# fbergama/wass

Hardware: AMD Instinct MI355X
Metric: stereo_pairs_per_sec (higher is better)
Workload: dtype u16

## Files before the change

### wass_amd/build.py

```python
from __future__ import annotations

import glob
import os
import subprocess
import sys

_HERE = os.path.dirname(os.path.abspath(__file__))
CSRC = os.path.join(_HERE, "csrc")
OBJ = os.path.join(CSRC, "_obj")
SO = os.path.join(_HERE, "libwassgpu.so")
HIPCC = os.environ.get("HIPCC", "/opt/rocm/bin/hipcc")
FLAGS = ["--offload-arch=gfx950", "-O3", "-std=c++17", "-fPIC", "-ffp-contract=off", "-Wall",
         "-Wno-unused-function", "-fno-gpu-rdc"] + os.environ.get("WASS_EXTRA_FLAGS", "").split()


def _newer(src: str, dst: str, deps) -> bool:
    if not os.path.exists(dst):
        return True
    t = os.path.getmtime(dst)
    return any(os.path.getmtime(p) > t for p in [src, *deps])


def build(force: bool = False, verbose: bool = False) -> str:
    os.makedirs(OBJ, exist_ok=True)
    srcs = sorted(glob.glob(os.path.join(CSRC, "*.hip")))
    deps = sorted(glob.glob(os.path.join(CSRC, "*.h"))) + [os.path.join(_HERE, "..", "include", "wass_gpu.h")]
    stamp = os.path.join(OBJ, ".flags")
    try:
        hipcc_version = subprocess.run([HIPCC, "--version"], capture_output=True, text=True).stdout.strip().replace("\n", " | ")
    except OSError:
        hipcc_version = "?"
    flags_now = " ".join(FLAGS) + " || " + hipcc_version
    try:
        same = open(stamp).read() == flags_now
    except OSError:
        same = False
    if not same:
        force = True
        for stale in (stamp, SO):
            try:
                os.remove(stale)
            except OSError:
                pass
    objs, procs = [], []
    for s in srcs:
        o = os.path.join(OBJ, os.path.basename(s)[:-4] + ".o")
        objs.append(o)
        if force or _newer(s, o, deps):
            cmd = [HIPCC, *FLAGS, "-c", s, "-o", o]
            if verbose:
                print(" ".join(cmd))
            procs.append((s, subprocess.Popen(cmd)))
    failed = [s for s, p in procs if p.wait() != 0]
    if failed:
        raise RuntimeError("hipcc failed for: " + ", ".join(failed))
    if force or procs or not os.path.exists(SO):
        cmd = [HIPCC, "--offload-arch=gfx950", "-shared", "-fPIC", "-o", SO, *objs, "-ldl"]
        if verbose:
            print(" ".join(cmd))
        subprocess.check_call(cmd)
    with open(stamp, "w") as f:
        f.write(flags_now)
    return SO


HOST_DIR = os.path.join(_HERE, "host")
BIN_DIR = os.path.join(_HERE, "bin")
CLI = os.path.join(BIN_DIR, "wass_stereo")
CLI_GPU = os.path.join(BIN_DIR, "wass_stereo_gpu")
BATCH = os.path.join(BIN_DIR, "wass_stereo_batch")
PREPARE = os.path.join(BIN_DIR, "wass_prepare")


def build_host(force: bool = False, verbose: bool = False) -> str:
    build(force=False)
    os.makedirs(BIN_DIR, exist_ok=True)
    deps = sorted(glob.glob(os.path.join(HOST_DIR, "*.hpp"))) + [os.path.join(_HERE, "..", "include", "wass_gpu.h"), SO]
    for name, exe in (("wass_stereo_client.cpp", CLI), ("wass_stereo.cpp", CLI_GPU), ("wass_stereo_batch.cpp", BATCH), ("wass_prepare.cpp", PREPARE)):
        src = os.path.join(HOST_DIR, name)
        if force or _newer(src, exe, deps):
            cmd = [os.environ.get("CXX", "g++"), "-O2", "-std=c++17", "-Wall", "-Wno-unused-function", src, "-o", exe]
            if exe != CLI:
                cmd += ["-L" + _HERE, "-lwassgpu", "-lz", "-pthread", "-Wl,-rpath,$ORIGIN/..", "-Wl,-rpath-link," + "/opt/rocm/lib"]
            if verbose:
                print(" ".join(cmd))
            subprocess.check_call(cmd)
    return CLI


if __name__ == "__main__":
    print(build(force="--force" in sys.argv, verbose=True))
    print(build_host(force="--force" in sys.argv, verbose=True))
```

### wass_amd/csrc/sgm_aggregate.hip

```cpp
#include "sgm_step.h"

namespace wass {

template <int NP, int SMODE, int U>
__global__ void __launch_bounds__(256) k_sweep(const uint32_t* __restrict__ C, uint32_t* __restrict__ S,
                                               int width1, int h, int dx, int dy, int P1, int P2, int nchains, int D,
                                               int minD, int uniq, int keepS, int16_t* __restrict__ sel_d16,
                                               uint32_t* __restrict__ sel_key)
{
    const int lane = threadIdx.x & 63;
    const int c = blockIdx.x * 4 + __builtin_amdgcn_readfirstlane(threadIdx.x >> 6);
    if (c >= nchains) return;
    int x0, y0, n;
    chain_geometry(c, dx, dy, width1, h, x0, y0, n);
    const long long vec = 64 * NP;
    const long long step = ((long long)dy * width1 + dx) * vec;
    const long long pixstep = (long long)dy * width1 + dx;
    long long pix = (long long)y0 * width1 + x0;
    const uint32_t* cp = C + pix * vec + lane * NP;
    uint32_t* sp = S + pix * vec + lane * NP;
    const us2 P1v = pk_splat(P1), cap = pk_splat(0x7FFF);

    auto finish = [&](const us2 (&L)[NP], const us2 (&sin)[NP], uint32_t* so, us2 (&sv)[NP]) {
#pragma unroll
        for (int j = 0; j < NP; ++j) sv[j] = SMODE == 0 ? pk_min(L[j], cap) : pk_min(pk_adds(sin[j], L[j]), cap);
        if (SMODE != 2 || keepS) {
            st_stream_vec<NP>(so, sv);
        }
    };

    PathState<NP> st;
    st.reset();
    const int F = n / U, r = n - F * U;
    us2 cb[U][NP], sb[U][NP], cn[U][NP], sn[U][NP];
    if (F > 0) {
        load_seg<NP, U, false>(cp, step, U, cb);
        if (SMODE != 0) load_seg<NP, U, false>(sp, step, U, sb);
    }
    for (int g = 0; g < F; ++g) {
        if (g + 1 < F) {
            load_seg<NP, U, false>(cp + U * step, step, U, cn);
            if (SMODE != 0) load_seg<NP, U, false>(sp + U * step, step, U, sn);
        }
        us2 fin[U][NP];
#pragma unroll
        for (int u = 0; u < U; ++u) {
            us2 L[NP];
            sgm_step<NP>(st, cb[u], L, P1v, P2);
            finish(L, sb[u], sp + u * step, fin[u]);
        }
        if (SMODE == 2) wta_batch<NP, U>(fin, U, lane, D, minD, uniq, sel_d16, sel_key, pix, pixstep);
        copy_seg<NP, U>(cb, cn);
        if (SMODE != 0) copy_seg<NP, U>(sb, sn);
        cp += U * step;
        sp += U * step;
        pix += U * pixstep;
    }
    if (r > 0) {
        load_seg<NP, U, true>(cp, step, r, cb);
        if (SMODE != 0) load_seg<NP, U, true>(sp, step, r, sb);
        us2 fin[U][NP];
#pragma unroll
        for (int u = 0; u < U; ++u) {
#pragma unroll
            for (int j = 0; j < NP; ++j) fin[u][j] = cap;
            if (u < r) {
                us2 L[NP];
                sgm_step<NP>(st, cb[u], L, P1v, P2);
                finish(L, sb[u], sp + u * step, fin[u]);
            }
        }
        if (SMODE == 2) wta_batch<NP, U>(fin, r, lane, D, minD, uniq, sel_d16, sel_key, pix, pixstep);
    }
}

#ifndef WASS_CKPT_WAVES
#define WASS_CKPT_WAVES 3
#endif
template <int NP, int K>
__global__ void __launch_bounds__(256) __attribute__((amdgpu_waves_per_eu(1, WASS_CKPT_WAVES))) k_ckpt(const uint32_t* __restrict__ C, uint32_t* __restrict__ ckpt,
                                              uint16_t* __restrict__ mins, int width1, int h, int dx, int dy, int P1, int P2,
                                              int nchains, int maxseg, uint32_t* __restrict__ endstate)
{
    const int lane = threadIdx.x & 63;
    const int c = blockIdx.x * 4 + __builtin_amdgcn_readfirstlane(threadIdx.x >> 6);
    if (c >= nchains) return;
    int x0, y0, n;
    if (endstate) half_chain_geometry(c, dx, dy, width1, h, x0, y0, n);
    else chain_geometry(c, dx, dy, width1, h, x0, y0, n);
    constexpr int VB = 256 * NP;
    const long long vec = 64 * NP;
    ChainAddr a;
    a.pixstep = (long long)dy * width1 + dx;
    a.pix0 = (long long)y0 * width1 + x0;
    a.sstep = (int)a.pixstep * VB;
    const uint32_t voff = lane * NP * 4;
    const uint32_t bK = a.bias(K);
    const us2 P1v = pk_splat(P1);
    const int F = n / K, r = n - F * K;
    const int ncp = endstate ? F : F - (r > 0 ? 0 : 1);
    const rsrc_t ckr = mk_rsrc(ckpt + (long long)c * maxseg * vec);
    uint32_t* mrow = (uint32_t*)(mins + (size_t)c * maxseg * K);

    PathState<NP> st;
    st.reset();
    us2 ring[K][NP];
    if (ncp > 0) {
        const rsrc_t r0 = a.run<NP>(C, 0, K);
#pragma unroll
        for (int u = 0; u < K; ++u) buf_ld<NP>(r0, voff, bK + u * a.sstep, ring[u]);
    }
    for (int s = 0; s < ncp; ++s) {
        uint32_t ms[K];
        const rsrc_t rn = a.run<NP>(C, (long long)min(s + 1, F - 1) * K, K);
#pragma unroll
        for (int u = 0; u < K; ++u) {
            us2 L[NP];
            sgm_step<NP>(st, ring[u], L, P1v, P2);
            ms[u] = st.m;
            buf_ld<NP>(rn, voff, bK + u * a.sstep, ring[u]);
        }
        {
            const us2 mvv = pk_splat(st.m);
            us2 nrm[NP];
#pragma unroll
            for (int j = 0; j < NP; ++j) nrm[j] = st.L[j] - mvv;
            buf_st<NP>(ckr, voff, (uint32_t)s * VB, nrm);
        }
        store_minima<K>(mrow + (size_t)s * (K / 2), ms, lane);
    }
    if (endstate) {
        if (r > 0) {
            const rsrc_t rt = a.run<NP>(C, (long long)F * K, r);
            const uint32_t br = a.bias(r);
#pragma unroll
            for (int u = 0; u < K; ++u)
                if (u < r) buf_ld<NP>(rt, voff, br + u * a.sstep, ring[u]);
#pragma unroll
            for (int u = 0; u < K; ++u)
                if (u < r) {
                    us2 L[NP];
                    sgm_step<NP>(st, ring[u], L, P1v, P2);
                }
        }
        st.store_normalised(endstate + (long long)c * vec + lane * NP);
    }
}

template <int NP>
__device__ __forceinline__ void lds_st(uint32_t* p, const us2 (&v)[NP])
{
    if constexpr (NP % 4 == 0) {
#pragma unroll
        for (int j = 0; j < NP; j += 4) *(wass_u32x4*)(p + j) = wass_u32x4{ as_u32(v[j]), as_u32(v[j + 1]), as_u32(v[j + 2]), as_u32(v[j + 3]) };
    } else if constexpr (NP % 2 == 0) {
#pragma unroll
        for (int j = 0; j < NP; j += 2) *(wass_u32x2*)(p + j) = wass_u32x2{ as_u32(v[j]), as_u32(v[j + 1]) };
    } else {
#pragma unroll
        for (int j = 0; j < NP; ++j) p[j] = as_u32(v[j]);
    }
}
template <int NP>
__device__ __forceinline__ void lds_ld(const uint32_t* p, us2 (&v)[NP])
{
    if constexpr (NP % 4 == 0) {
#pragma unroll
        for (int j = 0; j < NP; j += 4) {
            const wass_u32x4 t = *(const wass_u32x4*)(p + j);
            v[j] = as_us2(t.x); v[j + 1] = as_us2(t.y); v[j + 2] = as_us2(t.z); v[j + 3] = as_us2(t.w);
        }
    } else if constexpr (NP % 2 == 0) {
#pragma unroll
        for (int j = 0; j < NP; j += 2) {
            const wass_u32x2 t = *(const wass_u32x2*)(p + j);
            v[j] = as_us2(t.x); v[j + 1] = as_us2(t.y);
        }
    } else {
#pragma unroll
        for (int j = 0; j < NP; ++j) v[j] = as_us2(p[j]);
    }
}

#ifndef WASS_VREC
#define WASS_VREC 7
#endif
#ifndef WASS_REC_TIE
#define WASS_REC_TIE 0
#endif
#ifndef WASS_REC_FENCE
#define WASS_REC_FENCE 1
#endif
template <int N, bool VEC>
struct Rec {
    uint32_t v[VEC ? 1 : N / 2];
    __device__ __forceinline__ void clear()
    {
#pragma unroll
        for (int i = 0; i < (VEC ? 1 : N / 2); ++i) v[i] = 0;
    }
    __device__ __forceinline__ void load(const uint32_t* p, int lane)
    {
        if constexpr (VEC) {
            v[0] = __builtin_amdgcn_raw_buffer_load_b32(mk_rsrc(p), (uint32_t)min(lane, N / 2 - 1) * 4u, 0, 0);
#if WASS_REC_TIE
            asm volatile("" : "+v"(v[0]) :: "memory");
#elif WASS_REC_FENCE
            asm volatile("" ::: "memory");
#endif
        } else {
#pragma unroll
            for (int i = 0; i < N / 2; ++i) v[i] = p[i];
        }
    }
    __device__ __forceinline__ uint32_t at(int i) const
    {
        if constexpr (VEC) return (__builtin_amdgcn_readlane(v[0], i >> 1) >> ((i & 1) * 16)) & 0xFFFFu;
        else return (v[i >> 1] >> ((i & 1) * 16)) & 0xFFFFu;
    }
    __device__ __forceinline__ uint32_t at_dyn(int i) const
    {
        uint32_t w;
        if constexpr (VEC) w = __builtin_amdgcn_readlane(v[0], i >> 1);
        else {
            w = v[0];
#pragma unroll
            for (int k = 1; k < N / 2; ++k) w = (i >> 1) == k ? v[k] : w;
        }
        return (w >> ((i & 1) * 16)) & 0xFFFFu;
    }
    __device__ __forceinline__ uint32_t before(int u) const { return u == 0 ? 0u : at(u - 1); }
};

#ifndef WASS_PAIR_WAVES
#define WASS_PAIR_WAVES 4
#endif
template <int NP, int K, int SMODE>
__global__ void __launch_bounds__(256) __attribute__((amdgpu_waves_per_eu(WASS_PAIR_WAVES, WASS_PAIR_WAVES)))
k_pair(const uint32_t* __restrict__ C, uint32_t* __restrict__ S, const uint32_t* __restrict__ ckpt,
       const uint16_t* __restrict__ mins, int width1, int h, int dx, int dy, int P1, int P2, int nchains, int maxseg, int D,
       int minD, int uniq, int keepS, int16_t* __restrict__ sel_d16, uint32_t* __restrict__ sel_key,
       const uint32_t* __restrict__ endstate)
{
    static_assert(K % 2 == 0, "the minima records are read as dwords");
    constexpr int VW = 64 * NP;
    __shared__ __attribute__((aligned(16))) uint32_t hand[4][2][K][VW];
    const int lane = threadIdx.x & 63;
    const int wv = __builtin_amdgcn_readfirstlane(threadIdx.x >> 6);
    const int c = blockIdx.x * 4 + wv;
    if (c >= nchains) return;
    int x0, y0, n;
    if (endstate) half_chain_geometry(c, dx, dy, width1, h, x0, y0, n);
    else chain_geometry(c, dx, dy, width1, h, x0, y0, n);
    constexpr int VB = 256 * NP;
    constexpr bool LAST = SMODE == 2;
    const long long vec = VW;
    ChainAddr a;
    a.pixstep = (long long)dy * width1 + dx;
    a.pix0 = (long long)y0 * width1 + x0;
    a.sstep = (int)a.pixstep * VB;
    const uint32_t voff = lane * NP * 4;
    const uint32_t bK = a.bias(K);
    const us2 P1v = pk_splat(P1), cap = pk_splat(0x7FFF);
    const int F = n / K, r = n - F * K;
    const rsrc_t ckr = mk_rsrc(ckpt + (long long)c * maxseg * vec);
    const uint32_t* mrow = (const uint32_t*)(mins + (size_t)c * maxseg * K);
    uint32_t* hc = &hand[wv][0][0][lane * NP];
    uint32_t* hl = &hand[wv][1][0][lane * NP];

    PathState<NP> bw;
    bw.reset();
    if (endstate) {
        us2 nv[NP];
        ld_stream_vec<NP>(endstate + (long long)(c ^ 1) * vec + lane * NP, nv);
        bw.load_normalised(nv);
    }
    auto finish = [&](const us2 (&lf)[NP], const us2 (&lb)[NP], const us2 (&sin)[NP], us2 (&sv)[NP]) {
#pragma unroll
        for (int j = 0; j < NP; ++j) {
            const us2 both = pk_adds(lf[j], lb[j]);
            const us2 acc = SMODE == 0 ? both : pk_adds(sin[j], both);
            sv[j] = LAST ? pk_min(acc, cap) : acc;
        }
    };
    if (r > 0) {
        const rsrc_t rc = a.run<NP>(C, (long long)F * K, r), rs = a.run<NP>(S, (long long)F * K, r);
        const uint32_t br = a.bias(r);
        us2 cb[K][NP], lf[K][NP], sb[K][NP];
#pragma unroll
        for (int u = 0; u < K; ++u)
            if (u < r) {
                buf_ld<NP>(rc, voff, br + u * a.sstep, cb[u]);
                if (SMODE != 0) buf_ld<NP>(rs, voff, br + u * a.sstep, sb[u]);
            }
        PathState<NP> fw;
        fw.reset();
        if (F > 0) {
            us2 nv[NP];
            buf_ld<NP>(ckr, voff, (uint32_t)(F - 1) * VB, nv);
            fw.load_normalised(nv);
        }
#pragma unroll
        for (int u = 0; u < K; ++u)
            if (u < r) sgm_step<NP>(fw, cb[u], lf[u], P1v, P2);
        us2 fin[K][NP];
#pragma unroll
        for (int u = K - 1; u >= 0; --u) {
#pragma unroll
            for (int j = 0; j < NP; ++j) fin[u][j] = cap;
            if (u < r) {
                us2 L[NP];
                sgm_step<NP>(bw, cb[u], L, P1v, P2);
                finish(lf[u], L, sb[u], fin[u]);
                if (!LAST || keepS) buf_st<NP>(rs, voff, br + u * a.sstep, fin[u]);
            }
        }
        if (LAST) wta_batch<NP, K>(fin, r, lane, D, minD, uniq, sel_d16, sel_key, a.pix0 + (long long)F * K * a.pixstep, a.pixstep);
    }
    if (F == 0) return;

    us2 cf[K][NP], sr[K][NP];
    PathState<NP> fw;
    us2 nvB[NP];
    Rec<K, (WASS_VREC & 1) != 0> mB;
    mB.clear();
    {
        const int s = F - 1;
        const rsrc_t rc = a.run<NP>(C, (long long)s * K, K), rs = a.run<NP>(S, (long long)s * K, K);
        const rsrc_t rc2 = a.run<NP>(C, (long long)max(s - 1, 0) * K, K);
        if (s >= 2) buf_ld<NP>(ckr, voff, (uint32_t)(s - 2) * VB, nvB);
        else {
#pragma unroll
            for (int j = 0; j < NP; ++j) nvB[j] = pk_splat(0);
        }
        mB.load(mrow + (size_t)max(s - 1, 0) * (K / 2), lane);
        us2 c0[K][NP];
        fw.reset();
        us2 nv[NP];
        if (s >= 1) buf_ld<NP>(ckr, voff, (uint32_t)(s - 1) * VB, nv);
#pragma unroll
        for (int u = 0; u < K; ++u) {
            buf_ld<NP>(rc, voff, bK + u * a.sstep, c0[u]);
            if (SMODE != 0) buf_ld<NP>(rs, voff, bK + u * a.sstep, sr[u]);
        }
#pragma unroll
        for (int u = 0; u < K; ++u) buf_ld<NP>(rc2, voff, bK + u * a.sstep, cf[u]);
        if (s >= 1) fw.load_normalised(nv);
#pragma unroll
        for (int u = 0; u < K; ++u) {
            us2 L[NP];
            sgm_step<NP>(fw, c0[u], L, P1v, P2);
            lds_st<NP>(hc + u * VW, c0[u]);
            lds_st<NP>(hl + u * VW, L);
        }
    }

    us2 fin[K][NP];
    bool odd = false;
    int s = F - 1;
    __builtin_amdgcn_s_waitcnt(0x0F70);
    while (s >= 1) {
        const rsrc_t rcN = a.run<NP>(C, (long long)max(s - 2, 0) * K, K);
        const rsrc_t rsN = a.run<NP>(S, (long long)(s - 1) * K, K), rsO = a.run<NP>(S, (long long)s * K, K);
        us2 nvC[NP];
        Rec<K, (WASS_VREC & 1) != 0> mC;
        if (s >= 3) buf_ld<NP>(ckr, voff, (uint32_t)(s - 3) * VB, nvC);
        else {
#pragma unroll
            for (int j = 0; j < NP; ++j) nvC[j] = pk_splat(0);
        }
        mC.load(mrow + (size_t)max(s - 2, 0) * (K / 2), lane);
        fw.load_normalised(nvB);
        const int stp = odd ? VW : -VW;
        uint32_t* pc = hc + (odd ? 0 : (K - 1) * VW);
        us2 cbn[NP], lfn[NP];
        lds_ld<NP>(pc, cbn);
        lds_ld<NP>(pc + K * VW, lfn);
#pragma unroll
        for (int u = 0; u < K; ++u) {
            const int v = K - 1 - u;
            uint32_t* pn = pc + stp;
            us2 cb[NP], lfv[NP], Lf[NP], Lb[NP], sv[NP];
#pragma unroll
            for (int j = 0; j < NP; ++j) { cb[j] = cbn[j]; lfv[j] = lfn[j]; }
            if (u + 1 < K) {
                lds_ld<NP>(pn, cbn);
                lds_ld<NP>(pn + K * VW, lfn);
            }
            sgm_step_fb<NP>(fw, mB.before(u), cf[u], Lf, bw, cb, Lb, P1v, P2);
            finish(lfv, Lb, sr[v], sv);
            if (!LAST || keepS) buf_st<NP>(rsO, voff, bK + v * a.sstep, sv);
            if (LAST) {
#pragma unroll
                for (int j = 0; j < NP; ++j) fin[v][j] = sv[j];
            }
            lds_st<NP>(pc, cf[u]);
            lds_st<NP>(pc + K * VW, Lf);
            buf_ld<NP>(rcN, voff, bK + u * a.sstep, cf[u]);
            if (SMODE != 0) buf_ld<NP>(rsN, voff, bK + v * a.sstep, sr[v]);
            pc = pn;
        }
        if (LAST) wta_batch<NP, K>(fin, K, lane, D, minD, uniq, sel_d16, sel_key, a.pix0 + (long long)s * K * a.pixstep, a.pixstep);
#pragma unroll
        for (int j = 0; j < NP; ++j) nvB[j] = nvC[j];
        mB = mC;
        odd = !odd;
        --s;
    }
    {
        const rsrc_t rsO = a.run<NP>(S, 0, K);
        const int stp = odd ? VW : -VW;
        uint32_t* pc = hc + (odd ? 0 : (K - 1) * VW);
#pragma unroll
        for (int u = 0; u < K; ++u) {
            const int v = K - 1 - u;
            us2 cb[NP], lfv[NP], Lb[NP], sv[NP];
            lds_ld<NP>(pc, cb);
            lds_ld<NP>(pc + K * VW, lfv);
            sgm_step<NP>(bw, cb, Lb, P1v, P2);
            finish(lfv, Lb, sr[v], sv);
            if (!LAST || keepS) buf_st<NP>(rsO, voff, bK + v * a.sstep, sv);
            if (LAST) {
#pragma unroll
                for (int j = 0; j < NP; ++j) fin[v][j] = sv[j];
            }
            pc += stp;
        }
        if (LAST) wta_batch<NP, K>(fin, K, lane, D, minD, uniq, sel_d16, sel_key, a.pix0, a.pixstep);
    }
}

#ifndef WASS_FUSE_NP
#define WASS_FUSE_NP 4
#endif
template <int NP> struct Fuse {
    static constexpr int XB = NP <= 3 ? 10 : 8;
    static constexpr int MINW = NP <= 2 ? 5 : 2;
    static constexpr int MAXW = NP <= 2 ? 5 : (NP == 3 ? 3 : 2);
};
inline int fuse_xb(int NP) { return NP <= 3 ? 10 : 8; }

template <int NP>
__global__ void __launch_bounds__(256) __attribute__((amdgpu_waves_per_eu(1, 4)))
k_rowsweep(const uint32_t* __restrict__ C, uint32_t* __restrict__ entF, uint32_t* __restrict__ entB, uint16_t* __restrict__ MF,
           uint16_t* __restrict__ MB, int width1, int h, int P1, int P2, int nbx)
{
    constexpr int XB = Fuse<NP>::XB;
    const int lane = threadIdx.x & 63;
    const int y = blockIdx.x * 4 + __builtin_amdgcn_readfirstlane(threadIdx.x >> 6);
    if (y >= h) return;
    constexpr int VB = 256 * NP;
    const long long vec = 64 * NP;
    const int n = width1;
    ChainAddr af, ab;
    af.pixstep = 1;  af.pix0 = (long long)y * width1;           af.sstep = VB;
    ab.pixstep = -1; ab.pix0 = (long long)y * width1 + n - 1;   ab.sstep = -VB;
    const uint32_t voff = lane * NP * 4;
    const us2 P1v = pk_splat(P1);
    const int cb = n % XB;
    uint32_t* mfrow = (uint32_t*)(MF + (size_t)y * nbx * XB);
    uint16_t* mbrow = MB + (size_t)y * nbx * XB;
    uint32_t* efrow = entF + (size_t)y * nbx * vec + lane * NP;
    uint32_t* ebrow = entB + (size_t)y * nbx * vec + lane * NP;

    PathState<NP> sf, sb;
    sf.reset();
    sb.reset();
    us2 rf[XB][NP], rb[XB][NP];
    const int G = n / XB, rem = n - G * XB;
    if (G > 0) {
        const rsrc_t r0 = af.run<NP>(C, 0, XB), r1 = ab.run<NP>(C, 0, XB);
        const uint32_t b1 = ab.bias(XB);
#pragma unroll
        for (int u = 0; u < XB; ++u) {
            buf_ld<NP>(r0, voff, u * VB, rf[u]);
            buf_ld<NP>(r1, voff, b1 + u * ab.sstep, rb[u]);
        }
        __builtin_amdgcn_s_waitcnt(0x0F70);
    }
    for (int g = 0; g < G; ++g) {
        const int t0 = g * XB;
        const int nxt = min(t0 + XB, n - 1), cnn = min(XB, n - nxt);
        const rsrc_t rnf = af.run<NP>(C, nxt, cnn), rnb = ab.run<NP>(C, nxt, cnn);
        const uint32_t bnb = ab.bias(cnn);
        uint32_t msf[XB], msb[XB];
#pragma unroll
        for (int u = 0; u < XB; ++u) {
            const int t = t0 + u;
            if (u == 0 && g > 0) sf.store_normalised(efrow + (size_t)g * vec);
            if (u == cb && t > 0) sb.store_normalised(ebrow + (size_t)((n - 1 - t) / XB) * vec);
            us2 Lf[NP], Lb[NP];
            sgm_step_pair<NP>(sf, rf[u], Lf, sb, rb[u], Lb, P1v, P2);
            msf[u] = sf.m;
            msb[XB - 1 - u] = sb.m;
            const int uc = min(u, cnn - 1);
            buf_ld<NP>(rnf, voff, uc * VB, rf[u]);
            buf_ld<NP>(rnb, voff, bnb + uc * ab.sstep, rb[u]);
        }
        store_minima<XB>(mfrow + (size_t)g * (XB / 2), msf, lane);
        {
            uint32_t v = msb[0];
#pragma unroll
            for (int i = 1; i < XB; ++i) v = lane == i ? msb[i] : v;
            if (lane < XB) mbrow[n - t0 - XB + lane] = (uint16_t)v;
        }
    }
    if (rem > 0) {
        const int t0 = G * XB;
        if (G == 0) {
            const rsrc_t r0 = af.run<NP>(C, 0, rem), r1 = ab.run<NP>(C, 0, rem);
            const uint32_t b1 = ab.bias(rem);
#pragma unroll
            for (int u = 0; u < XB; ++u)
                if (u < rem) {
                    buf_ld<NP>(r0, voff, u * VB, rf[u]);
                    buf_ld<NP>(r1, voff, b1 + u * ab.sstep, rb[u]);
                }
        }
        uint32_t msf[XB], msb[XB];
#pragma unroll
        for (int i = 0; i < XB; ++i) msf[i] = msb[i] = 0;
#pragma unroll
        for (int u = 0; u < XB; ++u)
            if (u < rem) {
                const int t = t0 + u;
                if (u == 0 && G > 0) sf.store_normalised(efrow + (size_t)G * vec);
                if (u == cb && t > 0) sb.store_normalised(ebrow + (size_t)((n - 1 - t) / XB) * vec);
                us2 Lf[NP], Lb[NP];
                sgm_step_pair<NP>(sf, rf[u], Lf, sb, rb[u], Lb, P1v, P2);
                msf[u] = sf.m;
#pragma unroll
                for (int i = 0; i < XB; ++i) msb[i] = i == rem - 1 - u ? sb.m : msb[i];
            }
        store_minima<XB>(mfrow + (size_t)G * (XB / 2), msf, lane);
        {
            uint32_t v = msb[0];
#pragma unroll
            for (int i = 1; i < XB; ++i) v = lane == i ? msb[i] : v;
            if (lane < rem) mbrow[lane] = (uint16_t)v;
        }
    }
}

struct RowSide {
    const uint32_t* entF; const uint32_t* entB;
    const uint16_t* MF; const uint16_t* MB;
    int nbx;
};

template <int NP, int K, bool ACC, bool ONE>
__global__ void __launch_bounds__(64 * Fuse<NP>::XB) __attribute__((amdgpu_waves_per_eu(Fuse<NP>::MINW, Fuse<NP>::MAXW)))
k_pairx(const uint32_t* __restrict__ C, uint32_t* __restrict__ S, const uint32_t* __restrict__ ckpt, const uint16_t* __restrict__ mins,
        const RowSide rs, int width1, int h, int P1, int P2, int maxseg, const uint32_t* __restrict__ endstate)
{
    constexpr int XB = Fuse<NP>::XB;
    static_assert(K % 2 == 0 && K <= XB && XB % 2 == 0, "one wave per row of a K-row segment; minima records are read as dwords");
    static_assert((size_t)XB * 2 * K * 256 * NP <= 160 * 1024, "the hand-over block must fit a CU's LDS");
    constexpr int VW = 64 * NP, VB = 256 * NP;
    extern __shared__ __attribute__((aligned(16))) uint32_t hand_raw[];
    constexpr int SS = XB * VW;
    constexpr int KS = K * XB * VW;
    const int lane = threadIdx.x & 63;
    const int wv = __builtin_amdgcn_readfirstlane(threadIdx.x >> 6);
    const int bx = blockIdx.x >> 1, half = blockIdx.x & 1;
    const uint32_t keepF = (!ONE || half == 0) ? 0xFFFFFFFFu : 0u, keepB = (!ONE || half == 1) ? 0xFFFFFFFFu : 0u;
    auto drop = [](us2 (&v)[NP], uint32_t keep) {
        if constexpr (ONE) {
#pragma unroll
            for (int j = 0; j < NP; ++j) v[j] = as_us2(as_u32(v[j]) & keep);
        }
    };
    const int X0 = bx * XB, ncol = min(XB, width1 - X0);
    const bool colact = wv < ncol;
    const int x = colact ? X0 + wv : X0;
    const int c = 2 * x + half;
    int dx = 0, dy = 1, x0, y0, n;
    half_chain_geometry(c, dx, dy, width1, h, x0, y0, n);
    if (n == 0) return;
    const long long vec = VW;
    ChainAddr a;
    a.pixstep = (long long)dy * width1;
// ... 490 lines not shown
```

### wass_amd/csrc/sgm_step.h

```cpp
#pragma once

#include "common.h"

namespace wass {

#ifndef WASS_NT
#define WASS_NT 1
#endif
__device__ __forceinline__ uint32_t ld_stream(const uint32_t* p)
{
#if WASS_NT
    return __builtin_nontemporal_load(p);
#else
    return *p;
#endif
}
__device__ __forceinline__ void st_stream(uint32_t* p, uint32_t v)
{
#if WASS_NT
    __builtin_nontemporal_store(v, p);
#else
    *p = v;
#endif
}
// ... 227 lines not shown
}

template <int K>
__device__ __forceinline__ void store_minima(uint32_t* __restrict__ rec, const uint32_t (&ms)[K], int lane)
{
    static_assert(K % 2 == 0, "records are dwords");
    uint32_t v = ms[0] | (ms[1] << 16);
#pragma unroll
    for (int i = 1; i < K / 2; ++i) v = lane == i ? (ms[2 * i] | (ms[2 * i + 1] << 16)) : v;
    if (lane < K / 2) rec[lane] = v;
}

template <int NP>
__device__ __forceinline__ void sgm_step_fb(PathState<NP>& a, const uint32_t am, const us2 (&ca)[NP], us2 (&La)[NP],
                                            PathState<NP>& b, const us2 (&cb)[NP], us2 (&Lb)[NP],
                                            const us2 P1v, const uint32_t P2)
{
    a.shr = dpp_mov<DPP_WAVE_SHR1>(a.shr, as_u32(a.L[NP - 1]));
    b.shr = dpp_mov<DPP_WAVE_SHR1>(b.shr, as_u32(b.L[NP - 1]));
    a.shl = dpp_mov<DPP_WAVE_SHL1>(a.shl, as_u32(a.L[0]));
    b.shl = dpp_mov<DPP_WAVE_SHL1>(b.shl, as_u32(b.L[0]));
    const us2 amv = pk_splat(am), amp2 = pk_splat(am + P2);
    const us2 bmv = pk_splat(b.m), bmp2 = pk_splat(b.m + P2);
#pragma unroll
    for (int j = 0; j < NP; ++j) {
        const uint32_t alo = j == 0 ? a.shr : as_u32(a.L[j - 1]);
        const uint32_t blo = j == 0 ? b.shr : as_u32(b.L[j - 1]);
        const uint32_t ahi = j == NP - 1 ? a.shl : as_u32(a.L[j + 1]);
        const uint32_t bhi = j == NP - 1 ? b.shl : as_u32(b.L[j + 1]);
        const us2 anl = as_us2(__builtin_amdgcn_alignbit(as_u32(a.L[j]), alo, 16));
        const us2 bnl = as_us2(__builtin_amdgcn_alignbit(as_u32(b.L[j]), blo, 16));
        const us2 anr = as_us2(__builtin_amdgcn_alignbit(ahi, as_u32(a.L[j]), 16));
        const us2 bnr = as_us2(__builtin_amdgcn_alignbit(bhi, as_u32(b.L[j]), 16));
        us2 ax = pk_min(anl, anr);
        us2 bx = pk_min(bnl, bnr);
        ax = pk_adds(ax, P1v);
        bx = pk_adds(bx, P1v);
        ax = pk_min(a.L[j], ax);
        bx = pk_min(b.L[j], bx);
        ax = pk_min(ax, amp2);
        bx = pk_min(bx, bmp2);
        ax = ax - amv;
        bx = bx - bmv;
        La[j] = pk_adds(ca[j], ax);
        Lb[j] = pk_adds(cb[j], bx);
    }
    us2 bm = Lb[0];
#pragma unroll
    for (int j = 1; j < NP; ++j) bm = pk_min(bm, Lb[j]);
    b.m = wave_min_u32(min((uint32_t)bm.x, (uint32_t)bm.y));
#pragma unroll
    for (int j = 0; j < NP; ++j) { a.L[j] = La[j]; b.L[j] = Lb[j]; }
}

template <int NP>
__device__ __forceinline__ void sgm_step_ff(PathState<NP>& a, const uint32_t am, const us2 (&ca)[NP], us2 (&La)[NP],
                                            PathState<NP>& b, const uint32_t bm, const us2 (&cb)[NP], us2 (&Lb)[NP],
                                            const us2 P1v, const uint32_t P2)
{
    a.shr = dpp_mov<DPP_WAVE_SHR1>(a.shr, as_u32(a.L[NP - 1]));
    b.shr = dpp_mov<DPP_WAVE_SHR1>(b.shr, as_u32(b.L[NP - 1]));
    a.shl = dpp_mov<DPP_WAVE_SHL1>(a.shl, as_u32(a.L[0]));
    b.shl = dpp_mov<DPP_WAVE_SHL1>(b.shl, as_u32(b.L[0]));
    const us2 amv = pk_splat(am), amp2 = pk_splat(am + P2);
    const us2 bmv = pk_splat(bm), bmp2 = pk_splat(bm + P2);
#pragma unroll
    for (int j = 0; j < NP; ++j) {
        const uint32_t alo = j == 0 ? a.shr : as_u32(a.L[j - 1]);
        const uint32_t blo = j == 0 ? b.shr : as_u32(b.L[j - 1]);
        const uint32_t ahi = j == NP - 1 ? a.shl : as_u32(a.L[j + 1]);
        const uint32_t bhi = j == NP - 1 ? b.shl : as_u32(b.L[j + 1]);
        const us2 anl = as_us2(__builtin_amdgcn_alignbit(as_u32(a.L[j]), alo, 16));
        const us2 bnl = as_us2(__builtin_amdgcn_alignbit(as_u32(b.L[j]), blo, 16));
        const us2 anr = as_us2(__builtin_amdgcn_alignbit(ahi, as_u32(a.L[j]), 16));
        const us2 bnr = as_us2(__builtin_amdgcn_alignbit(bhi, as_u32(b.L[j]), 16));
        us2 ax = pk_min(anl, anr);
        us2 bx = pk_min(bnl, bnr);
        ax = pk_adds(ax, P1v);
        bx = pk_adds(bx, P1v);
        ax = pk_min(a.L[j], ax);
        bx = pk_min(b.L[j], bx);
        ax = pk_min(ax, amp2);
        bx = pk_min(bx, bmp2);
        ax = ax - amv;
        bx = bx - bmv;
        La[j] = pk_adds(ca[j], ax);
        Lb[j] = pk_adds(cb[j], bx);
    }
#pragma unroll
    for (int j = 0; j < NP; ++j) { a.L[j] = La[j]; b.L[j] = Lb[j]; }
}
template <int NP>
__device__ __forceinline__ void sgm_step_f(PathState<NP>& a, const uint32_t am, const us2 (&ca)[NP], us2 (&La)[NP], const us2 P1v,
                                           const uint32_t P2)
{
    a.shr = dpp_mov<DPP_WAVE_SHR1>(a.shr, as_u32(a.L[NP - 1]));
    a.shl = dpp_mov<DPP_WAVE_SHL1>(a.shl, as_u32(a.L[0]));
    const us2 amv = pk_splat(am), amp2 = pk_splat(am + P2);
#pragma unroll
    for (int j = 0; j < NP; ++j) {
        const uint32_t alo = j == 0 ? a.shr : as_u32(a.L[j - 1]);
        const uint32_t ahi = j == NP - 1 ? a.shl : as_u32(a.L[j + 1]);
        const us2 anl = as_us2(__builtin_amdgcn_alignbit(as_u32(a.L[j]), alo, 16));
        const us2 anr = as_us2(__builtin_amdgcn_alignbit(ahi, as_u32(a.L[j]), 16));
        us2 ax = pk_adds(pk_min(anl, anr), P1v);
        ax = pk_min(pk_min(a.L[j], ax), amp2) - amv;
        La[j] = pk_adds(ca[j], ax);
    }
#pragma unroll
    for (int j = 0; j < NP; ++j) a.L[j] = La[j];
}

__device__ __forceinline__ void chain_geometry(int c, int dx, int dy, int width1, int h, int& x0, int& y0, int& n)
{
    if (dy == 0) { y0 = c; x0 = dx > 0 ? 0 : width1 - 1; n = width1; }
    else if (dx == 0) { x0 = c; y0 = dy > 0 ? 0 : h - 1; n = h; }
    else {
        if (c < width1) { x0 = c; y0 = dy > 0 ? 0 : h - 1; }
        else { const int k = c - width1 + 1; x0 = dx > 0 ? 0 : width1 - 1; y0 = dy > 0 ? k : h - 1 - k; }
        const int nx = dx > 0 ? width1 - x0 : x0 + 1;
        const int ny = dy > 0 ? h - y0 : y0 + 1;
        n = min(nx, ny);
    }
}

__device__ __forceinline__ void half_chain_geometry(int c2, int& dx, int& dy, int width1, int h, int& x0, int& y0, int& n)
{
    chain_geometry(c2 >> 1, dx, dy, width1, h, x0, y0, n);
    const int mid = n / 2;
    if (c2 & 1) { x0 += (n - 1) * dx; y0 += (n - 1) * dy; dx = -dx; dy = -dy; n -= mid; }
    else n = mid;
}

template <int NP, int K, bool GUARD>
__device__ __forceinline__ void load_seg(const uint32_t* __restrict__ p, long long step, int len, us2 (&dst)[K][NP])
{
#pragma unroll
    for (int u = 0; u < K; ++u)
        if (!GUARD || u < len) {
            ld_stream_vec<NP>(p + u * step, dst[u]);
        }
}

template <int NP, int K>
__device__ __forceinline__ void copy_seg(us2 (&dst)[K][NP], const us2 (&src)[K][NP])
{
#pragma unroll
    for (int u = 0; u < K; ++u)
#pragma unroll
        for (int j = 0; j < NP; ++j) dst[u][j] = src[u][j];
}

template <int NP>
__device__ __forceinline__ int s_at(const us2 (&Sv)[NP], int d)
{
    const int ln = d / (2 * NP), slot = d % (2 * NP);
    uint32_t pv = 0;
#pragma unroll
    for (int j = 0; j < NP; ++j) {
        const uint32_t w = (uint32_t)__builtin_amdgcn_readlane((int)as_u32(Sv[j]), ln);
        pv = (slot >> 1) == j ? w : pv;
    }
    return (int)((slot & 1) ? (pv >> 16) : (pv & 0xFFFF));
}

__device__ __forceinline__ int div_small(int num, int den)
{
    const int an = num < 0 ? -num : num;
    int q = (int)((float)an * __builtin_amdgcn_rcpf((float)den));
    const int r = an - q * den;
    q += (r >= den) - (r < 0);
    return num < 0 ? -q : q;
}

#ifndef WASS_WTA_VECTOR_TAIL
#define WASS_WTA_VECTOR_TAIL 1
#endif
#if WASS_WTA_VECTOR_TAIL
template <int NP, int K>
__device__ __forceinline__ void wta_batch_eval(const us2 (&Sv)[K][NP], int lane, int D, int minD, int uniq, int& res_d,
                                               uint32_t& res_k)
{
    constexpr int V = 2 * NP;
    constexpr int ABSENT = 1 << 22;
    const int dlane = lane * V;
    uint32_t key[K];
#pragma unroll
    for (int u = 0; u < K; ++u) {
        key[u] = 0xFFFFFFFFu;
#pragma unroll
        for (int j = 0; j < NP; ++j) {
            const uint32_t w = as_u32(Sv[u][j]);
            key[u] = min(key[u], min((w << 16) | (uint32_t)(dlane + 2 * j), (w & 0xFFFF0000u) | (uint32_t)(dlane + 2 * j + 1)));
        }
    }
#pragma unroll
    for (int u = 0; u < K; ++u) key[u] = wave_min_u32(key[u]);
    const int q = 100 - uniq;
    unsigned long long inr[V];
#pragma unroll
    for (int j = 0; j < V; ++j) {
        const int nl = (D - j + V - 1) / V;
        inr[j] = nl >= 64 ? ~0ull : ((1ull << (nl < 0 ? 0 : nl)) - 1ull);
    }
    uint32_t g_key = 0xFFFFFFFFu, g_aw[NP], g_cw[NP];
    int g_cnt = 0;
#pragma unroll
    for (int j = 0; j < NP; ++j) g_aw[j] = g_cw[j] = 0;
#pragma unroll
    for (int u = 0; u < K; ++u) {
        const int minS = (int)(key[u] >> 16);
        const int best = minS >= 32767 ? -1 : (int)(key[u] & 0xFFFF);
        const int T = minS * 100;
        int cnt = 0;
#pragma unroll
        for (int j = 0; j < V; ++j) {
            const uint32_t sv = (j & 1) ? Sv[u][j >> 1].y : Sv[u][j >> 1].x;
            cnt += __builtin_popcountll(__builtin_amdgcn_ballot_w64((int)__umul24(sv, (uint32_t)q) < T) & inr[j]);
        }
        const int lna = max(best - 1, 0) / V, lnc = min(best + 1, D - 1) / V;
        const bool mine = lane == u;
        g_key = mine ? key[u] : g_key;
        g_cnt = mine ? cnt : g_cnt;
#pragma unroll
        for (int j = 0; j < NP; ++j) {
            const uint32_t aw = (uint32_t)__builtin_amdgcn_readlane((int)as_u32(Sv[u][j]), lna);
            const uint32_t cw = (uint32_t)__builtin_amdgcn_readlane((int)as_u32(Sv[u][j]), lnc);
            g_aw[j] = mine ? aw : g_aw[j];
            g_cw[j] = mine ? cw : g_cw[j];
        }
    }
    const int minS = (int)(g_key >> 16);
    const int best = minS >= 32767 ? -1 : (int)(g_key & 0xFFFF);
    const int T = minS * 100;
    auto half_at = [&](const uint32_t (&w)[NP], int d) {
        const int slot = d % V;
        uint32_t pv = 0;
#pragma unroll
        for (int j = 0; j < NP; ++j) pv = (slot >> 1) == j ? w[j] : pv;
        return (int)((slot & 1) ? (pv >> 16) : (pv & 0xFFFF));
    };
    const int am = half_at(g_aw, max(best - 1, 0)), cp = half_at(g_cw, min(best + 1, D - 1));
    const int a = best >= 1 ? am : ABSENT, cc = best + 1 < D ? cp : ABSENT;
    const int near = (a * q < T) + (cc * q < T) + (best >= 0 && minS * q < T);
    const bool ok = g_cnt <= near, sub = 0 < best && best < D - 1;
    const int denom2 = max(a + cc - 2 * minS, 1);
    const int frac = div_small((a - cc) * 16 + denom2, denom2 * 2);
    res_d = ok ? (best * 16 + (sub ? frac : 0) + minD * 16) : (minD - 1) * 16;
    res_k = ok ? (((uint32_t)minS << 16) | (uint32_t)(best & 0xFFFF)) : 0xFFFFFFFFu;
}
#else
template <int NP, int K>
__device__ __forceinline__ void wta_batch_eval(const us2 (&Sv)[K][NP], int lane, int D, int minD, int uniq, int& res_d,
                                               uint32_t& res_k)
{
    constexpr int V = 2 * NP;
    constexpr int ABSENT = 1 << 22;
    const int dlane = lane * V;
    uint32_t key[K];
#pragma unroll
    for (int u = 0; u < K; ++u) {
        key[u] = 0xFFFFFFFFu;
#pragma unroll
        for (int j = 0; j < NP; ++j) {
            const uint32_t w = as_u32(Sv[u][j]);
            key[u] = min(key[u], min((w << 16) | (uint32_t)(dlane + 2 * j), (w & 0xFFFF0000u) | (uint32_t)(dlane + 2 * j + 1)));
        }
    }
#pragma unroll
    for (int u = 0; u < K; ++u) key[u] = wave_min_u32(key[u]);
    const int q = 100 - uniq;
    unsigned long long inr[V];
#pragma unroll
    for (int j = 0; j < V; ++j) {
        const int nl = (D - j + V - 1) / V;
        inr[j] = nl >= 64 ? ~0ull : ((1ull << (nl < 0 ? 0 : nl)) - 1ull);
    }
    res_d = 0;
    res_k = 0;
#pragma unroll
    for (int u = 0; u < K; ++u) {
        const int minS = (int)(key[u] >> 16);
        const int best = minS >= 32767 ? -1 : (int)(key[u] & 0xFFFF);
        const int T = minS * 100;
        int cnt = 0;
#pragma unroll
        for (int j = 0; j < V; ++j) {
            const uint32_t sv = (j & 1) ? Sv[u][j >> 1].y : Sv[u][j >> 1].x;
            cnt += __builtin_popcountll(__builtin_amdgcn_ballot_w64((int)__umul24(sv, (uint32_t)q) < T) & inr[j]);
        }
        const int am = s_at<NP>(Sv[u], max(best - 1, 0)), cp = s_at<NP>(Sv[u], min(best + 1, D - 1));
        const int a = best >= 1 ? am : ABSENT, cc = best + 1 < D ? cp : ABSENT;
        const int near = (a * q < T) + (cc * q < T) + (best >= 0 && minS * q < T);
        const bool ok = cnt <= near, sub = 0 < best && best < D - 1;
        const int denom2 = max(a + cc - 2 * minS, 1);
        const int frac = div_small((a - cc) * 16 + denom2, denom2 * 2);
        const int out = ok ? (best * 16 + (sub ? frac : 0) + minD * 16) : (minD - 1) * 16;
        const uint32_t k = ok ? (((uint32_t)minS << 16) | (uint32_t)(best & 0xFFFF)) : 0xFFFFFFFFu;
        res_d = lane == u ? out : res_d;
        res_k = lane == u ? k : res_k;
    }
}

#endif

template <int NP, int K>
__device__ __forceinline__ void wta_batch(const us2 (&Sv)[K][NP], int nvalid, int lane, int D, int minD, int uniq,
                                          int16_t* __restrict__ out_d16, uint32_t* __restrict__ out_key, long long pix0,
                                          long long pixstep)
{
    int res_d;
    uint32_t res_k;
    wta_batch_eval<NP, K>(Sv, lane, D, minD, uniq, res_d, res_k);
    if (lane < nvalid) {
        const long long px = pix0 + lane * pixstep;
        out_d16[px] = (int16_t)res_d;
        out_key[px] = res_k;
    }
}

template <int NP>
__device__ __forceinline__ void wta_select(const us2 (&Sv)[NP], int lane, int D, int minD, int uniq,
                                           int16_t* __restrict__ out_d16, uint32_t* __restrict__ out_key)
{
    us2 one[1][NP];
#pragma unroll
    for (int j = 0; j < NP; ++j) one[0][j] = Sv[j];
    wta_batch<NP, 1>(one, 1, lane, D, minD, uniq, out_d16, out_key, 0, 0);
}


}
```

Measured before the change: 123.0.

## Add LDS-transposed winner-take-all selection path for small disparity vectors in sweeps

Adds a transposed WTA evaluation that writes batches of aggregated cost vectors to LDS scratch and reads them back so each lane group holds a contiguous run of disparities. Min, count and neighbour lookups then use DPP group reductions instead of per-pixel ballots and readlanes. It is enabled by default in the final sweep kernel, and a second library variant enables it in the pair kernel. It costs extra LDS per workgroup and a store/load round trip per pass.

New measurement: 123.6 (median of 3 runs). About the same (+0.5%).

```diff
diff --git a/wass_amd/build.py b/wass_amd/build.py
--- a/wass_amd/build.py
+++ b/wass_amd/build.py
@@ -9,6 +9,7 @@
 CSRC = os.path.join(_HERE, "csrc")
 OBJ = os.path.join(CSRC, "_obj")
 SO = os.path.join(_HERE, "libwassgpu.so")
+SO_WTA_ALT = os.path.join(_HERE, "libwassgpu_wta_alt.so")
 HIPCC = os.environ.get("HIPCC", "/opt/rocm/bin/hipcc")
 FLAGS = ["--offload-arch=gfx950", "-O3", "-std=c++17", "-fPIC", "-ffp-contract=off", "-Wall",
          "-Wno-unused-function", "-fno-gpu-rdc"] + os.environ.get("WASS_EXTRA_FLAGS", "").split()
@@ -51,14 +52,23 @@
             if verbose:
                 print(" ".join(cmd))
             procs.append((s, subprocess.Popen(cmd)))
+    s = os.path.join(CSRC, "sgm_aggregate.hip")
+    o = os.path.join(OBJ, "sgm_aggregate_wta_alt.o")
+    objs0 = [o if x == os.path.join(OBJ, "sgm_aggregate.o") else x for x in objs]
+    if force or _newer(s, o, deps):
+        cmd = [HIPCC, *FLAGS, "-DWASS_WTA_TRANSPOSED=2", "-c", s, "-o", o]
+        if verbose:
+            print(" ".join(cmd))
+        procs.append((s, subprocess.Popen(cmd)))
     failed = [s for s, p in procs if p.wait() != 0]
     if failed:
         raise RuntimeError("hipcc failed for: " + ", ".join(failed))
-    if force or procs or not os.path.exists(SO):
-        cmd = [HIPCC, "--offload-arch=gfx950", "-shared", "-fPIC", "-o", SO, *objs, "-ldl"]
-        if verbose:
-            print(" ".join(cmd))
-        subprocess.check_call(cmd)
+    for so, oo in ((SO, objs), (SO_WTA_ALT, objs0)):
+        if force or procs or not os.path.exists(so):
+            cmd = [HIPCC, "--offload-arch=gfx950", "-shared", "-fPIC", "-o", so, *oo, "-ldl"]
+            if verbose:
+                print(" ".join(cmd))
+            subprocess.check_call(cmd)
     with open(stamp, "w") as f:
         f.write(flags_now)
     return SO
diff --git a/wass_amd/csrc/sgm_aggregate.hip b/wass_amd/csrc/sgm_aggregate.hip
--- a/wass_amd/csrc/sgm_aggregate.hip
+++ b/wass_amd/csrc/sgm_aggregate.hip
@@ -10,6 +10,9 @@
 {
     const int lane = threadIdx.x & 63;
     const int c = blockIdx.x * 4 + __builtin_amdgcn_readfirstlane(threadIdx.x >> 6);
+    constexpr bool TSEL = SMODE == 2 && wta_transposed<NP, U, WTA_IN_SWEEP>();
+    __shared__ __attribute__((aligned(16))) uint32_t wsel[TSEL ? 4 : 1][TSEL ? WtaLayout<NP>::SCRATCH_DW : 1];
+    uint32_t* const wscr = TSEL ? wsel[c & 3] : nullptr;
     if (c >= nchains) return;
     int x0, y0, n;
     chain_geometry(c, dx, dy, width1, h, x0, y0, n);
@@ -49,7 +52,7 @@
             sgm_step<NP>(st, cb[u], L, P1v, P2);
             finish(L, sb[u], sp + u * step, fin[u]);
         }
-        if (SMODE == 2) wta_batch<NP, U>(fin, U, lane, D, minD, uniq, sel_d16, sel_key, pix, pixstep);
+        if (SMODE == 2) wta_batch<NP, U, WTA_IN_SWEEP>(fin, U, lane, D, minD, uniq, sel_d16, sel_key, pix, pixstep, wscr);
         copy_seg<NP, U>(cb, cn);
         if (SMODE != 0) copy_seg<NP, U>(sb, sn);
         cp += U * step;
@@ -70,7 +73,7 @@
                 finish(L, sb[u], sp + u * step, fin[u]);
             }
         }
-        if (SMODE == 2) wta_batch<NP, U>(fin, r, lane, D, minD, uniq, sel_d16, sel_key, pix, pixstep);
+        if (SMODE == 2) wta_batch<NP, U, WTA_IN_SWEEP>(fin, r, lane, D, minD, uniq, sel_d16, sel_key, pix, pixstep, wscr);
     }
 }
 
@@ -147,41 +150,6 @@
     }
 }
 
-template <int NP>
-__device__ __forceinline__ void lds_st(uint32_t* p, const us2 (&v)[NP])
-{
-    if constexpr (NP % 4 == 0) {
-#pragma unroll
-        for (int j = 0; j < NP; j += 4) *(wass_u32x4*)(p + j) = wass_u32x4{ as_u32(v[j]), as_u32(v[j + 1]), as_u32(v[j + 2]), as_u32(v[j + 3]) };
-    } else if constexpr (NP % 2 == 0) {
-#pragma unroll
-        for (int j = 0; j < NP; j += 2) *(wass_u32x2*)(p + j) = wass_u32x2{ as_u32(v[j]), as_u32(v[j + 1]) };
-    } else {
-#pragma unroll
-        for (int j = 0; j < NP; ++j) p[j] = as_u32(v[j]);
-    }
-}
-template <int NP>
-__device__ __forceinline__ void lds_ld(const uint32_t* p, us2 (&v)[NP])
-{
-    if constexpr (NP % 4 == 0) {
-#pragma unroll
-        for (int j = 0; j < NP; j += 4) {
-            const wass_u32x4 t = *(const wass_u32x4*)(p + j);
-            v[j] = as_us2(t.x); v[j + 1] = as_us2(t.y); v[j + 2] = as_us2(t.z); v[j + 3] = as_us2(t.w);
-        }
-    } else if constexpr (NP % 2 == 0) {
-#pragma unroll
-        for (int j = 0; j < NP; j += 2) {
-            const wass_u32x2 t = *(const wass_u32x2*)(p + j);
-            v[j] = as_us2(t.x); v[j + 1] = as_us2(t.y);
-        }
-    } else {
-#pragma unroll
-        for (int j = 0; j < NP; ++j) v[j] = as_us2(p[j]);
-    }
-}
-
 #ifndef WASS_VREC
 #define WASS_VREC 7
 #endif
@@ -245,8 +213,14 @@
     static_assert(K % 2 == 0, "the minima records are read as dwords");
     constexpr int VW = 64 * NP;
     __shared__ __attribute__((aligned(16))) uint32_t hand[4][2][K][VW];
+    constexpr bool TSEL = SMODE == 2 && wta_transposed<NP, K, WTA_IN_PAIR>();
+    __shared__ __attribute__((aligned(16))) uint32_t wsel[TSEL ? 4 : 1][TSEL ? WtaLayout<NP>::SCRATCH_DW : 1];
+    constexpr size_t LDS_CU = 160 * 1024, HAND_WG = sizeof(hand), ALL_WG = HAND_WG + (TSEL ? sizeof(wsel) : 0);
+    static_assert(ALL_WG <= 64 * 1024, "static LDS of a workgroup");
+    static_assert(LDS_CU / ALL_WG >= (LDS_CU / HAND_WG < WASS_PAIR_WAVES ? LDS_CU / HAND_WG : WASS_PAIR_WAVES), "the selection's scratch must not cost a workgroup per CU");
     const int lane = threadIdx.x & 63;
     const int wv = __builtin_amdgcn_readfirstlane(threadIdx.x >> 6);
+    uint32_t* const wscr = TSEL ? wsel[wv] : nullptr;
     const int c = blockIdx.x * 4 + wv;
     if (c >= nchains) return;
     int x0, y0, n;
@@ -315,7 +289,7 @@
                 if (!LAST || keepS) buf_st<NP>(rs, voff, br + u * a.sstep, fin[u]);
             }
         }
-        if (LAST) wta_batch<NP, K>(fin, r, lane, D, minD, uniq, sel_d16, sel_key, a.pix0 + (long long)F * K * a.pixstep, a.pixstep);
+        if (LAST) wta_batch<NP, K, WTA_IN_PAIR>(fin, r, lane, D, minD, uniq, sel_d16, sel_key, a.pix0 + (long long)F * K * a.pixstep, a.pixstep, wscr);
     }
     if (F == 0) return;
 
@@ -400,7 +374,7 @@
             if (SMODE != 0) buf_ld<NP>(rsN, voff, bK + v * a.sstep, sr[v]);
             pc = pn;
         }
-        if (LAST) wta_batch<NP, K>(fin, K, lane, D, minD, uniq, sel_d16, sel_key, a.pix0 + (long long)s * K * a.pixstep, a.pixstep);
+        if (LAST) wta_batch<NP, K, WTA_IN_PAIR>(fin, K, lane, D, minD, uniq, sel_d16, sel_key, a.pix0 + (long long)s * K * a.pixstep, a.pixstep, wscr);
 #pragma unroll
         for (int j = 0; j < NP; ++j) nvB[j] = nvC[j];
         mB = mC;
@@ -426,7 +400,7 @@
             }
             pc += stp;
         }
-        if (LAST) wta_batch<NP, K>(fin, K, lane, D, minD, uniq, sel_d16, sel_key, a.pix0, a.pixstep);
+        if (LAST) wta_batch<NP, K, WTA_IN_PAIR>(fin, K, lane, D, minD, uniq, sel_d16, sel_key, a.pix0, a.pixstep, wscr);
     }
 }
 
diff --git a/wass_amd/csrc/sgm_step.h b/wass_amd/csrc/sgm_step.h
--- a/wass_amd/csrc/sgm_step.h
+++ b/wass_amd/csrc/sgm_step.h
@@ -403,6 +403,41 @@
 }
 
 template <int NP>
+__device__ __forceinline__ void lds_st(uint32_t* p, const us2 (&v)[NP])
+{
+    if constexpr (NP % 4 == 0) {
+#pragma unroll
+        for (int j = 0; j < NP; j += 4) *(wass_u32x4*)(p + j) = wass_u32x4{ as_u32(v[j]), as_u32(v[j + 1]), as_u32(v[j + 2]), as_u32(v[j + 3]) };
+    } else if constexpr (NP % 2 == 0) {
+#pragma unroll
+        for (int j = 0; j < NP; j += 2) *(wass_u32x2*)(p + j) = wass_u32x2{ as_u32(v[j]), as_u32(v[j + 1]) };
+    } else {
+#pragma unroll
+        for (int j = 0; j < NP; ++j) p[j] = as_u32(v[j]);
+    }
+}
+template <int NP>
+__device__ __forceinline__ void lds_ld(const uint32_t* p, us2 (&v)[NP])
+{
+    if constexpr (NP % 4 == 0) {
+#pragma unroll
+        for (int j = 0; j < NP; j += 4) {
+            const wass_u32x4 t = *(const wass_u32x4*)(p + j);
+            v[j] = as_us2(t.x); v[j + 1] = as_us2(t.y); v[j + 2] = as_us2(t.z); v[j + 3] = as_us2(t.w);
+        }
+    } else if constexpr (NP % 2 == 0) {
+#pragma unroll
+        for (int j = 0; j < NP; j += 2) {
+            const wass_u32x2 t = *(const wass_u32x2*)(p + j);
+            v[j] = as_us2(t.x); v[j + 1] = as_us2(t.y);
+        }
+    } else {
+#pragma unroll
+        for (int j = 0; j < NP; ++j) v[j] = as_us2(p[j]);
+    }
+}
+
+template <int NP>
 __device__ __forceinline__ int s_at(const us2 (&Sv)[NP], int d)
 {
     const int ln = d / (2 * NP), slot = d % (2 * NP);
@@ -555,16 +590,118 @@
 
 #endif
 
+enum { WTA_IN_SWEEP = 1, WTA_IN_PAIR = 2 };
+#ifndef WASS_WTA_TRANSPOSED
+#define WASS_WTA_TRANSPOSED WTA_IN_SWEEP
+#endif
+template <int NP> struct WtaLayout {
+    static constexpr int P = NP == 1 ? 8 : (NP == 2 ? 4 : 0);
+    static constexpr int SCRATCH_DW = P * 64 * NP;
+};
+template <int NP, int K, int WHERE>
+constexpr bool wta_transposed() { return (WASS_WTA_TRANSPOSED & WHERE) != 0 && WtaLayout<NP>::P > 0 && K % WtaLayout<NP>::P == 0; }
+
+typedef wass_u32x4 wass_u32x4_alias __attribute__((may_alias));
+typedef uint32_t wass_u32_alias __attribute__((may_alias));
+
+template <int LP>
+__device__ __forceinline__ uint32_t group_min_u32(uint32_t v)
+{
+    static_assert(LP == 8 || LP == 16, "groups inside a DPP row");
+    v = min(v, dpp_mov<DPP_QUAD_XOR1>(0xFFFFFFFFu, v));
+    v = min(v, dpp_mov<DPP_QUAD_XOR2>(0xFFFFFFFFu, v));
+    v = min(v, dpp_mov<DPP_ROW_HALF_MIRROR>(0xFFFFFFFFu, v));
+    if constexpr (LP == 16) v = min(v, dpp_mov<DPP_ROW_MIRROR>(0xFFFFFFFFu, v));
+    return v;
+}
+template <int LP>
+__device__ __forceinline__ uint32_t group_sum_u32(uint32_t v)
+{
+    static_assert(LP == 8 || LP == 16, "groups inside a DPP row");
+    v += dpp_mov<DPP_QUAD_XOR1>(0u, v);
+    v += dpp_mov<DPP_QUAD_XOR2>(0u, v);
+    v += dpp_mov<DPP_ROW_HALF_MIRROR>(0u, v);
+    if constexpr (LP == 16) v += dpp_mov<DPP_ROW_MIRROR>(0u, v);
+    return v;
+}
+
 template <int NP, int K>
+__device__ __forceinline__ void wta_batch_eval_t(const us2 (&Sv)[K][NP], uint32_t* __restrict__ scr, int lane, int D, int minD,
+                                                 int uniq, int& res_d, uint32_t& res_k, int& cell)
+{
+    constexpr int P = WtaLayout<NP>::P, LP = 64 / P, RD = NP * P, R = 2 * RD, VW = 64 * NP, NPASS = K / P;
+    static_assert(RD % 4 == 0, "a lane's run is read with 128-bit LDS loads");
+    constexpr int ABSENT = 1 << 22;
+    const int sub = lane & (LP - 1), pp = lane / LP, d0 = sub * R;
+    const int q = 100 - uniq;
+    const int npad = min(max(d0 + R - D, 0), R);
+    uint32_t one = 0x00010001u;
+    asm("" : "+v"(one));
+    uint32_t g_key = 0xFFFFFFFFu;
+    int g_cnt = 0, g_a = 0, g_c = 0;
+#pragma unroll
+    for (int ps = 0; ps < NPASS; ++ps) {
+#pragma unroll
+        for (int p = 0; p < P; ++p) lds_st<NP>(scr + p * VW + lane * NP, Sv[ps * P + p]);
+        uint32_t w[RD];
+#pragma unroll
+        for (int i = 0; i < RD; i += 4) {
+            const wass_u32x4 t = *(const wass_u32x4_alias*)(scr + lane * RD + i);
+            w[i] = t.x; w[i + 1] = t.y; w[i + 2] = t.z; w[i + 3] = t.w;
+        }
+        uint32_t key = 0xFFFFFFFFu;
+#pragma unroll
+        for (int i = 0; i < RD; ++i) key = min(key, min((w[i] << 16) | (uint32_t)(2 * i), (w[i] & 0xFFFF0000u) | (uint32_t)(2 * i + 1)));
+        key = group_min_u32<LP>(key + (uint32_t)d0);
+        const int minS = (int)(key >> 16);
+        const int T = minS * 100;
+        int thr = min(div_small(T + max(q, 1) - 1, max(q, 1)), 0x8000);
+        if (q <= 0) thr = T > 0 ? 0x8000 : (q < 0 ? 1 : 0);
+        const bool complement = q < 0 && T == 0;
+        const us2 thrv = pk_splat((unsigned)thr);
+        us2 acc = pk_splat(0);
+#pragma unroll
+        for (int i = 0; i < RD; ++i) acc = acc + pk_min(pk_subs(thrv, as_us2(w[i])), as_us2(one));
+        const int below = (int)acc.x + (int)acc.y;
+        int cnt = complement ? R - npad - below : below - (thr > 0x7FFF ? npad : 0);
+        cnt = (int)group_sum_u32<LP>((uint32_t)cnt);
+        const int best = minS >= 32767 ? -1 : (int)(key & 0xFFFF);
+        const wass_u32_alias* sp = scr + pp * VW;
+        const int da = max(best - 1, 0), dc = min(best + 1, D - 1);
+        const int am = (int)((sp[da >> 1] >> ((da & 1) * 16)) & 0xFFFFu), cp = (int)((sp[dc >> 1] >> ((dc & 1) * 16)) & 0xFFFFu);
+        const bool mine = sub == ps;
+        g_key = mine ? key : g_key;
+        g_cnt = mine ? cnt : g_cnt;
+        g_a = mine ? am : g_a;
+        g_c = mine ? cp : g_c;
+    }
+    const int minS = (int)(g_key >> 16);
+    const int best = minS >= 32767 ? -1 : (int)(g_key & 0xFFFF);
+    const int T = minS * 100;
+    const int a = best >= 1 ? g_a : ABSENT, cc = best + 1 < D ? g_c : ABSENT;
+    const int near = (a * q < T) + (cc * q < T) + (best >= 0 && minS * q < T);
+    const bool ok = g_cnt <= near, sub1 = 0 < best && best < D - 1;
+    const int denom2 = max(a + cc - 2 * minS, 1);
+    const int frac = div_small((a - cc) * 16 + denom2, denom2 * 2);
+    res_d = ok ? (best * 16 + (sub1 ? frac : 0) + minD * 16) : (minD - 1) * 16;
+    res_k = ok ? (((uint32_t)minS << 16) | (uint32_t)(best & 0xFFFF)) : 0xFFFFFFFFu;
+    cell = sub < NPASS ? sub * P + pp : K;
+}
+
+template <int NP, int K, int WHERE>
 __device__ __forceinline__ void wta_batch(const us2 (&Sv)[K][NP], int nvalid, int lane, int D, int minD, int uniq,
                                           int16_t* __restrict__ out_d16, uint32_t* __restrict__ out_key, long long pix0,
-                                          long long pixstep)
-{
-    int res_d;
+                                          long long pixstep, uint32_t* __restrict__ scr)
+{
+    int res_d, cell;
     uint32_t res_k;
-    wta_batch_eval<NP, K>(Sv, lane, D, minD, uniq, res_d, res_k);
-    if (lane < nvalid) {
-        const long long px = pix0 + lane * pixstep;
+    if constexpr (wta_transposed<NP, K, WHERE>()) wta_batch_eval_t<NP, K>(Sv, scr, lane, D, minD, uniq, res_d, res_k, cell);
+    else {
+        wta_batch_eval<NP, K>(Sv, lane, D, minD, uniq, res_d, res_k);
+        cell = lane;
+    }
+    if (cell < nvalid) {
+        const long long px = pix0 + cell * pixstep;
         out_d16[px] = (int16_t)res_d;
         out_key[px] = res_k;
     }
@@ -577,8 +714,8 @@
     us2 one[1][NP];
 #pragma unroll
     for (int j = 0; j < NP; ++j) one[0][j] = Sv[j];
-    wta_batch<NP, 1>(one, 1, lane, D, minD, uniq, out_d16, out_key, 0, 0);
-}
-
-
-}
+    wta_batch<NP, 1, 0>(one, 1, lane, D, minD, uniq, out_d16, out_key, 0, 0, nullptr);
+}
+
+
+}
```
